# comprna/riser

Measured on NVIDIA B200. Metric: reads classified/sec (4 s chunks), higher is better.
Workload: dtype f16+e4m3

## Files before the change

### riser_b200/csrc/common.cuh

```cuda
#pragma once

#include <cuda_runtime.h>
#include <cuda_fp16.h>
#include <cuda_fp8.h>
#include <stdint.h>
#include <stdio.h>
#include <stdarg.h>

#include "../../include/riser_b200.h"

namespace riser {

inline char* err_buf() {
  static thread_local char buf[512] = {0};
  return buf;
}
inline int fail(int code, const char* fmt, ...) {
  va_list ap;
  va_start(ap, fmt);
  vsnprintf(err_buf(), 512, fmt, ap);
  va_end(ap);
  return code;
}
#define RISER_CUDA_TRY(expr)                                                              \
// ... 69 lines not shown
#define RISER_SPIN_NS 0
#endif
__device__ __forceinline__ void mbar_wait_relaxed(uint64_t* bar, uint32_t parity) {
  while (!mbar_try_wait(bar, parity)) {
    if (RISER_SPIN_NS > 0) __nanosleep(RISER_SPIN_NS);
  }
}

__device__ __forceinline__ void tma_prefetch_desc(const void* tmap) {
  asm volatile("prefetch.tensormap [%0];" ::"l"(reinterpret_cast<uint64_t>(tmap)) : "memory");
}
__device__ __forceinline__ void tma_load_2d(void* smem_dst, const void* tmap, uint64_t* bar,
                                            int32_t c0, int32_t c1) {
  asm volatile(
      "cp.async.bulk.tensor.2d.shared::cluster.global.mbarrier::complete_tx::bytes "
      "[%0], [%1, {%3, %4}], [%2];"
      ::"r"(smem_u32(smem_dst)), "l"(reinterpret_cast<uint64_t>(tmap)), "r"(smem_u32(bar)),
      "r"(c0), "r"(c1)
      : "memory");
}

__device__ __forceinline__ void bulk_prefetch_l2(const void* gsrc, uint32_t bytes) {
  asm volatile("cp.async.bulk.prefetch.L2.global [%0], %1;" ::"l"(reinterpret_cast<uint64_t>(gsrc)), "r"(bytes)
               : "memory");
}

__device__ __forceinline__ void bulk_load_1d(void* smem_dst, const void* gsrc, uint32_t bytes, uint64_t* bar) {
  asm volatile(
      "cp.async.bulk.shared::cluster.global.mbarrier::complete_tx::bytes [%0], [%1], %2, [%3];"
      ::"r"(smem_u32(smem_dst)), "l"(reinterpret_cast<uint64_t>(gsrc)), "r"(bytes), "r"(smem_u32(bar))
      : "memory");
}

__device__ __forceinline__ void tmem_alloc(uint32_t* smem_slot, uint32_t cols) {
  asm volatile("tcgen05.alloc.cta_group::1.sync.aligned.shared::cta.b32 [%0], %1;"
               ::"r"(smem_u32(smem_slot)), "r"(cols)
               : "memory");
}
__device__ __forceinline__ void tmem_relinquish() {
  asm volatile("tcgen05.relinquish_alloc_permit.cta_group::1.sync.aligned;" ::: "memory");
}
__device__ __forceinline__ void tmem_dealloc(uint32_t taddr, uint32_t cols) {
  asm volatile("tcgen05.dealloc.cta_group::1.sync.aligned.b32 %0, %1;" ::"r"(taddr), "r"(cols)
               : "memory");
}
__device__ __forceinline__ void tc_fence_before() {
  asm volatile("tcgen05.fence::before_thread_sync;" ::: "memory");
}
__device__ __forceinline__ void tc_fence_after() {
  asm volatile("tcgen05.fence::after_thread_sync;" ::: "memory");
}
__device__ __forceinline__ void umma_f16(uint32_t tmem_d, uint64_t desc_a, uint64_t desc_b,
                                         uint32_t idesc, uint32_t accumulate) {
  asm volatile(
      "{\n\t.reg .pred p;\n\t"
      "setp.ne.b32 p, %4, 0;\n\t"
      "tcgen05.mma.cta_group::1.kind::f16 [%0], %1, %2, %3, p;\n\t}\n"
      ::"r"(tmem_d), "l"(desc_a), "l"(desc_b), "r"(idesc), "r"(accumulate)
      : "memory");
}
__device__ __forceinline__ void umma_f8(uint32_t tmem_d, uint64_t desc_a, uint64_t desc_b,
                                        uint32_t idesc, uint32_t accumulate) {
  asm volatile(
      "{\n\t.reg .pred p;\n\t"
      "setp.ne.b32 p, %4, 0;\n\t"
      "tcgen05.mma.cta_group::1.kind::f8f6f4 [%0], %1, %2, %3, p;\n\t}\n"
// ... 202 lines not shown
```

### riser_b200/csrc/convnet.cu

```cuda
#include "common.cuh"

#include <cuda.h>

#include <algorithm>
#include <cmath>
#include <cstdio>
#include <cstdlib>
#include <cstring>
#include <memory>
#include <vector>

namespace riser {
namespace {

#ifndef RISER_DBG
#define RISER_DBG 0
#endif
#ifndef RISER_UNIFORM_ISSUE
#define RISER_UNIFORM_ISSUE 1
#endif
constexpr int kMaxLayers = 16;
constexpr int kBlockM = 128;
constexpr int kBlockK = 64;
constexpr int kMaxNTile = 256;
// ... 121 lines not shown
  int fused_prev = 0;
  Eo2Args eo2;
  size_t eo2_smem = 0;
  ConvArgs args;
  int n_supers_total = 0;
  int rows_per_super = 0;
  int flag_off = 0;
  size_t smem = 0;
};

}
}

struct riser_plan {
  const riser_model* model = nullptr;
  int B = 0, max_len = 0;
  int fuse_l0 = 0;
  uint8_t* flags = nullptr;
  riser::ActivityArgs activity;
  int chunk_reads = 0, n_chunked = 0;
  int Lmax[riser::kMaxLayers + 1];
  int Lp[riser::kMaxLayers + 1];
  size_t act_off[riser::kMaxLayers + 1];
  char* ws = nullptr;
  riser::LayerPlan layer[riser::kMaxLayers];
};

namespace riser {
namespace {

constexpr float kF8AScale = 1.f / 8.f;
constexpr float kF8LoScale = 512.f;
template <int N>
__device__ __forceinline__ void store_f8_planes(const float (&r)[N], const __half2 (&h)[N / 2], uint8_t* a8,
                                                int lo_stride) {
  uint32_t pa[N / 4], pl[N / 4];
#pragma unroll
  for (int j = 0; j < N / 4; ++j) {
    uint32_t wa[2], wl[2];
#pragma unroll
    for (int e = 0; e < 2; ++e) {
      const int c = 4 * j + 2 * e;
      const float2 back = __half22float2(h[c / 2]);
      wa[e] = __nv_cvt_float2_to_fp8x2(make_float2(r[c] * kF8AScale, r[c + 1] * kF8AScale), __NV_SATFINITE,
                                       __NV_E4M3);
      wl[e] = __nv_cvt_float2_to_fp8x2(make_float2((r[c] - back.x) * kF8LoScale, (r[c + 1] - back.y) * kF8LoScale),
                                       __NV_SATFINITE, __NV_E4M3);
    }
    pa[j] = wa[0] | (wa[1] << 16);
    pl[j] = wl[0] | (wl[1] << 16);
  }
  if (N == 8) {
    *reinterpret_cast<uint2*>(a8) = make_uint2(pa[0], pa[1]);
    *reinterpret_cast<uint2*>(a8 + lo_stride) = make_uint2(pl[0], pl[1]);
  } else {
#pragma unroll
    for (int j = 0; j < N / 16; ++j) {
      *reinterpret_cast<uint4*>(a8 + 16 * j) = make_uint4(pa[4 * j], pa[4 * j + 1], pa[4 * j + 2], pa[4 * j + 3]);
      *reinterpret_cast<uint4*>(a8 + lo_stride + 16 * j) =
          make_uint4(pl[4 * j], pl[4 * j + 1], pl[4 * j + 2], pl[4 * j + 3]);
    }
  }
}

__global__ void __launch_bounds__(256)
layer0_kernel(const float* __restrict__ x, int64_t ld_x, const int32_t* __restrict__ len0,
              const float* __restrict__ w, const float* __restrict__ bias, __half* __restrict__ out,
              int B, int Lp1, int cout, int cout_p, int planes, int f8) {
  __shared__ float sw[64 * 3];
  __shared__ float sb[64];
  for (int i = threadIdx.x; i < cout_p * 3; i += blockDim.x) sw[i] = (i < cout * 3) ? w[i] : 0.f;
  for (int i = threadIdx.x; i < cout_p; i += blockDim.x) sb[i] = (i < cout) ? bias[i] : 0.f;
  __syncthreads();
  const uint32_t groups = cout_p >> 3;
  const uint32_t total = static_cast<uint32_t>(B) * Lp1 * groups;
  for (uint32_t idx = blockIdx.x * blockDim.x + threadIdx.x; idx < total; idx += gridDim.x * blockDim.x) {
    const uint32_t r = idx / groups;
    const int c8 = static_cast<int>(idx - r * groups);
    const int b = static_cast<int>(r / static_cast<uint32_t>(Lp1));
    const int tp = static_cast<int>(r - static_cast<uint32_t>(b) * Lp1);
    const int L = len0[b];
    uint4* o = reinterpret_cast<uint4*>(out + static_cast<int64_t>(r) * cout_p * planes) + c8;
    uint8_t* o8 = reinterpret_cast<uint8_t*>(out) + static_cast<int64_t>(r) * cout_p * 4 + 2 * cout_p + c8 * 8;
    if (tp >= (L >> 1)) {
// ... 585 lines not shown
  }
  if (ms == 4) return pick_conv_planes<4, false, false, K32>(planes, wplanes);
  if (ms == 2) return pick_conv_planes<2, false, false, K32>(planes, wplanes);
  return pick_conv_planes<1, false, false, K32>(planes, wplanes);
}
template <bool K32>
ConvKernelFn pick_conv_f8(int ms, int resident) {
  if (resident) {
    if (ms == 4) return conv_tc_kernel<4, 1, 1, true, false, K32, true>;
    if (ms == 2) return conv_tc_kernel<2, 1, 1, true, false, K32, true>;
    return conv_tc_kernel<1, 1, 1, true, false, K32, true>;
  }
  if (ms == 4) return conv_tc_kernel<4, 1, 1, false, false, K32, true>;
  if (ms == 2) return conv_tc_kernel<2, 1, 1, false, false, K32, true>;
  return conv_tc_kernel<1, 1, 1, false, false, K32, true>;
}
ConvKernelFn pick_conv_kernel(int ms, int planes, int wplanes, int resident, int fused = 0, int k32 = 0,
                              int f8 = 0) {
  if (f8) return k32 ? pick_conv_f8<true>(ms, resident) : pick_conv_f8<false>(ms, resident);
  return k32 ? pick_conv_k<true>(ms, planes, wplanes, resident, fused)
             : pick_conv_k<false>(ms, planes, wplanes, resident, fused);
}

constexpr int kF2Pairs = 255;
#ifndef RISER_F2_CVT_WARPS
#define RISER_F2_CVT_WARPS 6
#endif
constexpr int kF2Threads = 576 + 32 * RISER_F2_CVT_WARPS;
constexpr uint32_t kF2A1Tile = 264 * 64;
constexpr uint32_t kF2A0Tile = 256 * 64;
constexpr int kF2N0 = 48;
constexpr int kF2D0Col = 256;
constexpr int kF2CvtThreads = 32 * RISER_F2_CVT_WARPS;
constexpr int kF2XStages = 4;
constexpr int kF2MaxLocalItems = 2048;
constexpr uint32_t kF2XStage = 260 * 16;

struct F2Smem {
  uint64_t w_full;
  uint64_t x_full[kF2XStages], x_empty[kF2XStages];
  uint64_t a0_full[2], a0_empty[2];
  uint64_t d0_full[2], d0_empty[2];
  uint64_t a1_full[2], a1_empty[2];
  uint64_t d1_full[2], d1_empty[2][2];
  uint32_t tmem_base;
  alignas(16) float bias[32];
  uint8_t my_flags[kF2MaxLocalItems];
};

struct F2Iter {
  const uint8_t* local;
  int i, item, n_items, step;
  __device__ __forceinline__ F2Iter(const uint8_t* l, int n) : local(l), i(0), item(blockIdx.x), n_items(n), step(gridDim.x) {}
  __device__ __forceinline__ int take() {
    while (item < n_items) {
      const int cur = item;
      const bool f = local ? (local[i] != 0) : true;
      item += step;
      ++i;
      if (f) return cur;
    }
    return -1;
  }
};

__device__ __forceinline__ uint32_t h2_bits(__half2 h) { return *reinterpret_cast<uint32_t*>(&h); }

template <int MODE>
__global__ void __launch_bounds__(kF2Threads, 1)
fused01_kernel(const __grid_constant__ CUtensorMap tm_b, const __grid_constant__ CUtensorMap tm_b8, const ConvArgs a) {
  extern __shared__ unsigned char smem_dyn[];
  unsigned char* base = smem_dyn + ((1024u - (smem_u32(smem_dyn) & 1023u)) & 1023u);
  constexpr bool F8 = (MODE == 3);
  constexpr bool KC = (MODE == 4);
  constexpr int PLANES = (MODE >= 2) ? 2 : 1;
  constexpr int WPLANES = (MODE == 1 || MODE == 2) ? 2 : 1;
  constexpr uint32_t kW1Bytes = KC ? 3 * 32 * 128 : (F8 ? 2 : WPLANES) * 3 * 32 * 64;
  constexpr uint32_t kB0Bytes = kF2N0 * 64;
  constexpr uint32_t kA1Stage = PLANES * 2 * kF2A1Tile;
  unsigned char* w1 = base;
  unsigned char* b0 = w1 + kW1Bytes;
  unsigned char* a0_ring = b0 + kB0Bytes;
  unsigned char* a1_ring = a0_ring + 2 * kF2A0Tile;
  unsigned char* x_ring = a1_ring + 2 * kA1Stage;
  F2Smem& s = *reinterpret_cast<F2Smem*>(x_ring + kF2XStages * kF2XStage);

  const int warp = uniform_warp_id();
  const int lane = threadIdx.x & 31;
  const int n_items = a.n_supers;
  const int n_pairs = a.rows_in >> 1;
  const uint8_t* flags0 = a.flags ? a.flags + a.super0 : nullptr;
  const uint8_t* flags_l = flags0 ? s.my_flags : nullptr;

  if (threadIdx.x == 0) {
    tma_prefetch_desc(&tm_b);
    mbar_init(&s.w_full, 1);
    for (int i = 0; i < kF2XStages; ++i) {
      mbar_init(&s.x_full[i], 1);
      mbar_init(&s.x_empty[i], kF2CvtThreads / 32);
    }
    for (int i = 0; i < 2; ++i) {
      mbar_init(&s.a0_full[i], kF2CvtThreads / 32);
      mbar_init(&s.a0_empty[i], 1);
      mbar_init(&s.d0_full[i], 1);
      mbar_init(&s.d0_empty[i], 4);
      mbar_init(&s.a1_full[i], 8);
      mbar_init(&s.a1_empty[i], 1);
      mbar_init(&s.d1_full[i], 1);
      mbar_init(&s.d1_empty[i][0], 4);
      mbar_init(&s.d1_empty[i][1], 4);
    }
    fence_mbar_init();
  }
  if (warp == 1) {
    tmem_alloc(&s.tmem_base, kTmemCols);
    tmem_relinquish();
  }
  for (uint32_t i = threadIdx.x; i < (2 * kF2A0Tile + 2 * kA1Stage + kF2XStages * kF2XStage) / 16; i += kF2Threads)
// ... 5 lines not shown
  if (threadIdx.x < kF2N0) {
    const int n = threadIdx.x, c = n % 24, odd = n / 24;
    float w[3] = {0.f, 0.f, 0.f}, bb = 0.f;
    if (c < a.cout0) {
      w[0] = a.w0[c * 3];
      w[1] = a.w0[c * 3 + 1];
      w[2] = a.w0[c * 3 + 2];
      bb = a.b0[c];
    }
    __half kh[4], kl[4];
#pragma unroll
    for (int k = 0; k < 4; ++k) kh[k] = kl[k] = __float2half_rn(0.f);
#pragma unroll
    for (int tap = 0; tap < 3; ++tap) {
      const __half h = __float2half_rn(w[tap]);
      kh[tap + odd] = h;
      kl[tap + odd] = __float2half_rn(w[tap] - __half2float(h));
    }
    const __half bh = __float2half_rn(bb), bl = __float2half_rn(bb - __half2float(bh));
    __half c0[8] = {kh[0], kh[1], kh[2], kh[3], kh[0], kh[1], kh[2], kh[3]};
    __half c1[8] = {kl[0], kl[1], kl[2], kl[3], bh, bl, __float2half_rn(0.f), __float2half_rn(0.f)};
    const int sw = (n >> 1) & 3;
    *reinterpret_cast<uint4*>(b0 + n * 64 + ((0 ^ sw) << 4)) = *reinterpret_cast<const uint4*>(c0);
    *reinterpret_cast<uint4*>(b0 + n * 64 + ((1 ^ sw) << 4)) = *reinterpret_cast<const uint4*>(c1);
  }
  asm volatile("fence.proxy.async.shared::cta;" ::: "memory");
  tc_fence_before();
  __syncthreads();
  tc_fence_after();
  const uint32_t tmem_base = s.tmem_base;

  if (warp == 0) {
    if (lane == 0) {
      mbar_arrive_expect_tx(&s.w_full, kW1Bytes);
      if (KC) {
        for (int tap = 0; tap < 3; ++tap) tma_load_2d(w1 + (2 - tap) * 4096, &tm_b, &s.w_full, 0, tap * a.cout_p);
      } else {
        for (int wp = 0; wp < WPLANES; ++wp)
          for (int tap = 0; tap < 3; ++tap)
            tma_load_2d(w1 + (wp * 3 + 2 - tap) * 2048, &tm_b, &s.w_full, 0, (wp * 3 + tap) * a.cout_p);
      }
      if (F8)
        for (int tap = 0; tap < 3; ++tap)
          tma_load_2d(w1 + (3 + 2 - tap) * 2048, &tm_b8, &s.w_full, 0, tap * a.cout_p);
      const int t_max = static_cast<int>(a.ld_x >> 2);
      F2Iter iter(flags_l, n_items);
      int k = 0;
      for (int item = iter.take(); item >= 0; item = iter.take(), ++k) {
        const int st = k % kF2XStages;
        mbar_wait(&s.x_empty[st], ((k / kF2XStages) & 1) ^ 1);
        unsigned char* dst = x_ring + st * kF2XStage;
        long long u_lo = static_cast<long long>(a.super0 + item) * kF2Pairs - 2;
        long long u_hi = u_lo + 258;
        const int i_lo = (u_lo < 0) ? static_cast<int>(-u_lo) - 2 : -2;
        if (u_lo < 0) u_lo = 0;
        if (u_hi > n_pairs - 1) u_hi = n_pairs - 1;
        uint32_t bytes[2] = {0, 0};
        const float* src[2] = {nullptr, nullptr};
        int slot[2] = {0, 0};
        if (u_hi >= u_lo) {
          const int b = static_cast<int>((static_cast<unsigned long long>(static_cast<uint32_t>(u_lo)) * a.pair_magic) >> 40);
          const int t0 = static_cast<int>(u_lo) - b * a.half_lp;
          const int n_total = static_cast<int>(u_hi - u_lo) + 1;
          const int n_first = min(n_total, a.half_lp - t0);
          const int n1 = max(0, min(n_first, t_max - t0));
          src[0] = a.x + static_cast<long long>(b) * a.ld_x + 4 * t0;
          slot[0] = i_lo + 2;
          bytes[0] = 16u * n1;
          const int n2 = max(0, min(n_total - n_first, t_max));
          src[1] = a.x + static_cast<long long>(b + 1) * a.ld_x;
          slot[1] = i_lo + 2 + n_first;
          bytes[1] = 16u * n2;
        }
        mbar_arrive_expect_tx(&s.x_full[st], bytes[0] + bytes[1]);
        if (bytes[0]) bulk_load_1d(dst + 16 * slot[0], src[0], bytes[0], &s.x_full[st]);
        if (bytes[1]) bulk_load_1d(dst + 16 * slot[1], src[1], bytes[1], &s.x_full[st]);
      }
    }
  } else if (warp == 1) {
    const bool leader = RISER_UNIFORM_ISSUE ? elect_one() : (lane == 0);
    if (RISER_UNIFORM_ISSUE || lane == 0) {
      mbar_wait(&s.w_full, 0);
      tc_fence_after();
      const uint32_t w1_addr = smem_u32(w1), b0_addr = smem_u32(b0);
      const uint32_t a0_addr = smem_u32(a0_ring), a1_addr = smem_u32(a1_ring);
      const uint32_t idesc0 = umma_idesc_f16(kBlockM, kF2N0);
      const uint32_t idesc64 = umma_idesc_f16(kBlockM, 64);
      const uint64_t db0 = sw_desc<true>(b0_addr);
      F2Iter iter(flags_l, n_items);
      int k0 = 0;
      auto issue_layer0 = [&]() {
        const int st = k0 & 1;
        mbar_wait(&s.a0_full[st], (k0 >> 1) & 1);
        tc_fence_after();
#pragma unroll
        for (int h = 0; h < 2; ++h) {
          mbar_wait(&s.d0_empty[h], (k0 & 1) ^ 1);
          tc_fence_after();
          if (leader) {
#pragma unroll
            for (int sub = 0; sub < 2; ++sub)
              umma_f16(tmem_base + kF2D0Col + (h * 2 + sub) * kF2N0,
                       sw_desc<true>(a0_addr + st * kF2A0Tile + sub * 128 * 64) + 2 * h, db0, idesc0, 0);
          }
          umma_commit_p(leader, &s.d0_full[h]);
        }
        umma_commit_p(leader, &s.a0_empty[st]);
        ++k0;
      };
      int cur = iter.take();
      if (cur >= 0) issue_layer0();
      int k1 = 0;
      while (cur >= 0) {
        const int nxt = iter.take();
        if (nxt >= 0) issue_layer0();
        const int st = k1 & 1;
        mbar_wait(&s.a1_full[st], (k1 >> 1) & 1);
        tc_fence_after();
        const uint32_t a1s = a1_addr + st * kA1Stage;
#pragma unroll
        for (int sub = 0; sub < 2; ++sub) {
          mbar_wait(&s.d1_empty[st][sub], ((k1 >> 1) & 1) ^ 1);
          tc_fence_after();
        }
        auto issue_group = [&](uint32_t a_tiles, uint32_t w_set, bool f8, bool first) {
          if (!leader) return;
#pragma unroll
          for (int tap = 0; tap < 3; ++tap) {
#pragma unroll
            for (int k = 0; k < 2; ++k) {
              const uint64_t db = sw_desc<true>(w_set + (2 - tap) * 2048) + 2 * k;
#pragma unroll
              for (int sub = 0; sub < 2; ++sub) {
#pragma unroll
                for (int pe = 0; pe < 2; ++pe) {
                  const int par = (pe == 0) ? ((tap == 1) ? 0 : 1) : ((tap == 1) ? 1 : 0);
                  const int shift = (pe == 0) ? ((tap == 2) ? 1 : 0) : ((tap == 0) ? 0 : 1);
                  const uint64_t da = sw_desc<true>(a_tiles + par * kF2A1Tile + (sub * 128 + shift) * 64) + 2 * k;
                  const uint32_t d = tmem_base + st * 128 + (2 * sub + pe) * 32;
                  if ((RISER_DBG & 1) && !(first && tap == 0 && k == 0)) continue;
                  if (f8) umma_f8(d, da, db, a.idesc, 1);
                  else umma_f16(d, da, db, a.idesc, !(first && tap == 0 && k == 0));
                }
              }
            }
          }
        };
        if (KC) {
          if (leader) {
#pragma unroll
            for (int k = 0; k < 4; ++k) {
              const uint64_t w21 = sw_desc<false>(w1_addr) + 2 * k;
              const uint64_t w10 = sw_desc<false>(w1_addr + 4096) + 2 * k;
              const uint64_t w0 = sw_desc<false>(w1_addr + 8192) + 2 * k;
#pragma unroll
              for (int sub = 0; sub < 2; ++sub) {
                const uint32_t e_rows = a1s + sub * 128 * 128, o_rows = e_rows + 2 * kF2A1Tile;
                const uint32_t d_even = tmem_base + st * 128 + 2 * sub * 32, d_odd = d_even + 32;
                umma_f16(d_even, sw_desc<false>(e_rows) + 2 * k, w10, idesc64, k != 0);
                umma_f16(d_even, sw_desc<false>(o_rows + 128) + 2 * k, w21, idesc64, 1);
                umma_f16(d_even, sw_desc<false>(o_rows) + 2 * k, w0, a.idesc, 1);
                umma_f16(d_odd, sw_desc<false>(e_rows + 128) + 2 * k, w21, a.idesc, 1);
              }
            }
          }
        } else {
#pragma unroll
        for (int wp = 0; wp < WPLANES; ++wp)
#pragma unroll
          for (int ap = 0; ap < ((wp == 0 && !F8) ? PLANES : 1); ++ap)
            issue_group(a1s + ap * 2 * kF2A1Tile, w1_addr + wp * 3 * 2048, false, wp == 0 && ap == 0);
        }
        if (F8)
          issue_group(a1s + 2 * kF2A1Tile, w1_addr + 3 * 2048, true, false);
        umma_commit_p(leader, &s.a1_empty[st]);
        umma_commit_p(leader, &s.d1_full[st]);
        ++k1;
        cur = nxt;
      }
    }
  } else if (warp < 2 + kF2CvtThreads / 32) {
    const int ct = (warp - 2) * 32 + lane;
    const __half2 one2 = __floats2half2_rn(1.f, 1.f);
    F2Iter iter(flags_l, n_items);
    int k = 0;
    for (int item = iter.take(); item >= 0; item = iter.take(), ++k) {
      const int st = k & 1;
      const int xst = k % kF2XStages;
      mbar_wait_relaxed(&s.x_full[xst], (k / kF2XStages) & 1);
      mbar_wait_relaxed(&s.a0_empty[st], ((k >> 1) & 1) ^ 1);
      unsigned char* tile = a0_ring + st * kF2A0Tile;
      const float* xs = reinterpret_cast<const float*>(x_ring + xst * kF2XStage) + 8;
      const long long u0 = static_cast<long long>(a.super0 + item) * kF2Pairs;
      for (int i = ct - 1; i <= 255 && !(RISER_DBG & 32); i += kF2CvtThreads) {
        const long long u = u0 + i;
        const bool inb = (u >= 0 && u < n_pairs);
        const uint32_t uu = inb ? static_cast<uint32_t>(u) : 0u;
        const int b = static_cast<int>((static_cast<unsigned long long>(uu) * a.pair_magic) >> 40);
        const int t4 = 4 * (static_cast<int>(uu) - b * a.half_lp);
        const int L = inb ? __ldg(a.len0 + b) : 0;
        const float4 x03 = *reinterpret_cast<const float4*>(xs + 4 * i);
        const float2 x01 = make_float2(x03.x, x03.y), x23 = make_float2(x03.z, x03.w);
        float xm1 = (t4 > 0) ? xs[4 * i - 1] : 0.f;
        float x4 = xs[4 * i + 4];
        const int half_len = L >> 1;
        const bool e_ok = (t4 >> 1) < half_len;
        const bool o_ok = (t4 >> 1) + 1 < half_len;
        float x2 = (t4 + 2 < L) ? x23.x : 0.f;
        if (t4 + 4 >= L) x4 = 0.f;
        auto clampf = [](float v) { return fminf(fmaxf(v, -65504.f), 65504.f); };
        const float v[6] = {clampf(xm1), clampf(x01.x), clampf(x01.y), clampf(x2), clampf(x23.y), clampf(x4)};
        __half2 hi[3], lo[3];
#pragma unroll
        for (int j = 0; j < 3; ++j) {
          hi[j] = __floats2half2_rn(v[2 * j], v[2 * j + 1]);
          const float2 back = __half22float2(hi[j]);
          lo[j] = __floats2half2_rn(v[2 * j] - back.x, v[2 * j + 1] - back.y);
        }
        if (i >= 0) {
          unsigned char* row = tile + i * 64;
          const int sw = (i >> 1) & 3;
          uint4 c0 = make_uint4(0, 0, 0, 0), c1 = make_uint4(0, 0, 0, 0);
          if (e_ok) {
            c0 = make_uint4(h2_bits(hi[0]), h2_bits(hi[1]), h2_bits(lo[0]), h2_bits(lo[1]));
            c1 = make_uint4(h2_bits(hi[0]), h2_bits(hi[1]), h2_bits(one2), 0u);
          }
          *reinterpret_cast<uint4*>(row + ((0 ^ sw) << 4)) = c0;
          *reinterpret_cast<uint4*>(row + ((1 ^ sw) << 4)) = c1;
        }
        if (i + 1 <= 255) {
          unsigned char* row = tile + (i + 1) * 64;
          const int sw = ((i + 1) >> 1) & 3;
          uint4 c2 = make_uint4(0, 0, 0, 0), c3 = make_uint4(0, 0, 0, 0);
          if (o_ok) {
            c2 = make_uint4(h2_bits(hi[1]), h2_bits(hi[2]), h2_bits(lo[1]), h2_bits(lo[2]));
            c3 = make_uint4(h2_bits(hi[1]), h2_bits(hi[2]), h2_bits(one2), 0u);
          }
          *reinterpret_cast<uint4*>(row + ((2 ^ sw) << 4)) = c2;
          *reinterpret_cast<uint4*>(row + ((3 ^ sw) << 4)) = c3;
        }
      }
      asm volatile("fence.proxy.async.shared::cta;" ::: "memory");
      __syncwarp();
      if (lane == 0) {
        mbar_arrive(&s.x_empty[xst]);
        mbar_arrive(&s.a0_full[st]);
      }
    }
  } else if (warp < 10 + kF2CvtThreads / 32) {
    const int q = warp & 3;
    const int h = (warp - 2 - kF2CvtThreads / 32) >> 2;
    F2Iter iter(flags_l, n_items);
    int k = 0;
    for (int item = iter.take(); item >= 0; item = iter.take(), ++k) {
      const int st = k & 1;
      mbar_wait_relaxed(&s.a1_empty[st], ((k >> 1) & 1) ^ 1);
      mbar_wait_relaxed(&s.d0_full[h], k & 1);
      tc_fence_after();
      unsigned char* tile_hi = a1_ring + st * kA1Stage + h * kF2A1Tile;
#pragma unroll
      for (int sub = 0; sub < 2; ++sub) {
        const uint32_t taddr = tmem_base + (static_cast<uint32_t>(32 * q) << 16) + kF2D0Col + (h * 2 + sub) * kF2N0;
        uint32_t e0[16], e1[8], o0[16], o1[8];
        if (RISER_DBG & 4) {
#pragma unroll
          for (int j = 0; j < 16; ++j) e0[j] = o0[j] = 0u;
#pragma unroll
          for (int j = 0; j < 8; ++j) e1[j] = o1[j] = 0u;
        } else {
        tmem_ld_32x16(taddr, e0);
        tmem_ld_32x16(taddr + 24, o0);
        }
        if (RISER_DBG & 4) {
        } else if (a.cout0 > 20) {
          tmem_ld_32x8(taddr + 16, e1);
          tmem_ld_32x8(taddr + 40, o1);
        } else {
#pragma unroll
          for (int j = 4; j < 8; ++j) e1[j] = o1[j] = 0u;
          tmem_ld_32x4(taddr + 16, e1);
          tmem_ld_32x4(taddr + 40, o1);
        }
        tmem_ld_wait();
        if (sub == 1) {
          tc_fence_before();
          __syncwarp();
          if (lane == 0) mbar_arrive(&s.d0_empty[h]);
        }
        if (RISER_DBG & 16) continue;
        const int row = sub * 128 + 32 * q + lane;
// ... 37 lines not shown
          }
#pragma unroll
          for (int c8 = 0; c8 < 3; ++c8)
            *reinterpret_cast<uint4*>(rp + 2 * kF2A1Tile + ((c8 ^ sw) << 4)) = *reinterpret_cast<const uint4*>(lv + 4 * c8);
        }
        if (F8) {
          uint32_t pa[6], pl[6];
#pragma unroll
          for (int j = 0; j < 6; ++j) {
            uint32_t wa[2], wl[2];
#pragma unroll
            for (int e = 0; e < 2; ++e) {
              const int c = 4 * j + 2 * e;
              const float2 back = __half22float2(hv[c / 2]);
              wa[e] = __nv_cvt_float2_to_fp8x2(make_float2(v[c] * kF8AScale, v[c + 1] * kF8AScale), __NV_SATFINITE,
                                               __NV_E4M3);
              wl[e] = __nv_cvt_float2_to_fp8x2(
                  make_float2((v[c] - back.x) * kF8LoScale, (v[c + 1] - back.y) * kF8LoScale), __NV_SATFINITE, __NV_E4M3);
            }
            pa[j] = wa[0] | (wa[1] << 16);
            pl[j] = wl[0] | (wl[1] << 16);
          }
          unsigned char* rp8 = rp + 2 * kF2A1Tile;
          *reinterpret_cast<uint4*>(rp8 + ((0 ^ sw) << 4)) = make_uint4(pa[0], pa[1], pa[2], pa[3]);
          *reinterpret_cast<uint4*>(rp8 + ((1 ^ sw) << 4)) = make_uint4(pa[4], pa[5], 0u, 0u);
          *reinterpret_cast<uint4*>(rp8 + ((2 ^ sw) << 4)) = make_uint4(pl[0], pl[1], pl[2], pl[3]);
          *reinterpret_cast<uint4*>(rp8 + ((3 ^ sw) << 4)) = make_uint4(pl[4], pl[5], 0u, 0u);
        }
      }
      asm volatile("fence.proxy.async.shared::cta;" ::: "memory");
      __syncwarp();
      if (lane == 0) mbar_arrive(&s.a1_full[st]);
    }
  } else {
    const int q = warp & 3;
    const int sub = (warp - 10 - kF2CvtThreads / 32) >> 2;
    const int row_elems = a.cout_p * a.out_planes;
    const int lo_off = (a.out_planes == 2 && !a.out_f8) ? a.cout_p : 0;
    const float inv_scale = a.w_inv_scale;
    F2Iter iter(flags_l, n_items);
    int k = 0;
    for (int item = iter.take(); item >= 0; item = iter.take(), ++k) {
      const int st = k & 1;
      const int j = sub * 128 + 32 * q + lane;
      const long long u = static_cast<long long>(a.super0 + item) * kF2Pairs + j;
      const bool ok = (j < kF2Pairs) && (u < n_pairs);
      const uint32_t uu = ok ? static_cast<uint32_t>(u) : 0u;
      const int b = static_cast<int>((static_cast<unsigned long long>(uu) * a.pair_magic) >> 40);
      const int tp = static_cast<int>(uu) - b * a.half_lp;
      const bool valid = ok && tp < (__ldg(a.len0 + b) >> a.shift);
      const bool writable = ok && tp < a.Lp_out;
      const int64_t out_row = a.out_eo ? static_cast<int64_t>(tp & 1) * a.n_pairs_out + static_cast<int64_t>(b) * a.half_lp_out + (tp >> 1)
                                       : static_cast<int64_t>(b) * a.Lp_out + tp;
      __half* orow = static_cast<__half*>(a.out) + out_row * row_elems;
      mbar_wait_relaxed(&s.d1_full[st], (k >> 1) & 1);
      tc_fence_after();
      const uint32_t taddr = tmem_base + (static_cast<uint32_t>(32 * q) << 16) + st * 128 + 2 * sub * 32;
      auto finish = [&](int c16, const float (&m)[16]) {
        if (!(writable && !((RISER_DBG & 2) && a.Lp_out > 0))) return;
        float r[16];
        if (valid) {
#pragma unroll
          for (int c4 = 0; c4 < 4; ++c4) {
            const float4 bb = *reinterpret_cast<const float4*>(&s.bias[c16 * 16 + c4 * 4]);
            const float bv[4] = {bb.x, bb.y, bb.z, bb.w};
#pragma unroll
            for (int e = 0; e < 4; ++e) {
              const int c = c4 * 4 + e;
              r[c] = fmaxf(fmaf(m[c], inv_scale, bv[e]), 0.f);
            }
          }
        } else {
#pragma unroll
          for (int c = 0; c < 16; ++c) r[c] = 0.f;
        }
        __half2 hv[8];
#pragma unroll
        for (int c = 0; c < 8; ++c) hv[c] = sat_half2(r[2 * c], r[2 * c + 1]);
        st_global_256(orow + c16 * 16, *reinterpret_cast<const uint4*>(hv), *reinterpret_cast<const uint4*>(hv + 4));
        if (lo_off) {
          __half2 lv[8];
#pragma unroll
          for (int c = 0; c < 8; ++c) {
            const float2 back = __half22float2(hv[c]);
            lv[c] = __floats2half2_rn(r[2 * c] - back.x, r[2 * c + 1] - back.y);
          }
          st_global_256(orow + lo_off + c16 * 16, *reinterpret_cast<const uint4*>(lv),
                        *reinterpret_cast<const uint4*>(lv + 4));
        }
        if (a.out_f8)
          store_f8_planes<16>(r, hv, reinterpret_cast<uint8_t*>(orow) + 2 * a.cout_p + c16 * 16, a.cout_p);
      };
      float m0[16];
      {
        uint32_t ve[16], vo[16];
        if (RISER_DBG & 8) {
#pragma unroll
          for (int j = 0; j < 16; ++j) ve[j] = vo[j] = 0u;
        } else {
          tmem_ld_32x16(taddr, ve);
          tmem_ld_32x16(taddr + 32, vo);
        }
        tmem_ld_wait();
#pragma unroll
        for (int j = 0; j < 16; ++j) m0[j] = fmaxf(__uint_as_float(ve[j]), __uint_as_float(vo[j]));
      }
      uint32_t ve1[16], vo1[16];
      if (RISER_DBG & 8) {
#pragma unroll
        for (int j = 0; j < 16; ++j) ve1[j] = vo1[j] = 0u;
      } else {
        tmem_ld_32x16(taddr + 16, ve1);
        tmem_ld_32x16(taddr + 32 + 16, vo1);
      }
      finish(0, m0);
      tmem_ld_wait();
      tc_fence_before();
      __syncwarp();
      if (lane == 0) mbar_arrive(&s.d1_empty[st][sub]);
#pragma unroll
      for (int j = 0; j < 16; ++j) m0[j] = fmaxf(__uint_as_float(ve1[j]), __uint_as_float(vo1[j]));
      finish(1, m0);
      __syncwarp();
    }
  }

  tc_fence_before();
  __syncthreads();
  if (warp == 1) {
    tc_fence_after();
    tmem_dealloc(tmem_base, kTmemCols);
  }
}

typedef void (*FusedKernelFn)(const CUtensorMap, const CUtensorMap, const ConvArgs);
FusedKernelFn pick_fused01(int mode) {
  if (mode == 0) return fused01_kernel<0>;
  if (mode == 1) return fused01_kernel<1>;
  if (mode == 2) return fused01_kernel<2>;
  if (mode == 4) return fused01_kernel<4>;
  return fused01_kernel<3>;
}
size_t fused01_smem(int planes, int wplanes) {
  return 1024 + static_cast<size_t>(wplanes) * 3 * 32 * 64 + kF2N0 * 64 + 2 * kF2A0Tile +
         2 * static_cast<size_t>(planes) * 2 * kF2A1Tile + kF2XStages * kF2XStage + sizeof(F2Smem) + 64;
}

constexpr uint32_t kEoTile = 136 * 64;

template <int MS, int PLANES, int WPLANES>
__global__ void __launch_bounds__(64 + 128 * kMaxEpiSets, 1)
conv_eo_kernel(const __grid_constant__ CUtensorMap tm_e, const __grid_constant__ CUtensorMap tm_o,
               const __grid_constant__ CUtensorMap tm_b, const ConvArgs a) {
  extern __shared__ unsigned char smem_dyn[];
  unsigned char* base = smem_dyn + ((1024u - (smem_u32(smem_dyn) & 1023u)) & 1023u);
  constexpr uint32_t kGroup = MS * PLANES * 2 * kEoTile;
  const uint32_t b_bytes = a.n_tile * 64;
  unsigned char* a_ring = base;
  unsigned char* b_region = base + static_cast<size_t>(a.a_stages) * kGroup;
  const size_t b_region_bytes = static_cast<size_t>(WPLANES) * a.k_blocks * 3 * b_bytes;
  ConvSmem& s = *reinterpret_cast<ConvSmem*>(b_region + b_region_bytes);

  const int warp = uniform_warp_id();
  const int lane = threadIdx.x & 31;
  const int n_items = a.n_supers;
  const int acc2 = a.acc_cols;

  if (warp == 0 && lane == 0) {
    tma_prefetch_desc(&tm_e);
    tma_prefetch_desc(&tm_o);
    tma_prefetch_desc(&tm_b);
    for (int i = 0; i < a.a_stages; ++i) {
      mbar_init(&s.a_full[i], 1);
      mbar_init(&s.a_empty[i], 1);
    }
    mbar_init(&s.w_full, 1);
    for (int i = 0; i < a.acc_stages; ++i) {
      mbar_init(&s.tmem_full[i], 1);
// ... 1276 lines not shown
            break;
          }
        }
      }
    } else {
      a.resident = 0;
      a.ms = (2 * a.acc_cols <= kTmemCols) ? max_ms : 1;
      if (max_ms == 2 && 4 * a.acc_cols <= kTmemCols && 2 * 4 * a_group1 + 3 * b_bytes <= avail &&
          env_int("RISER_CONV_MS4_STREAM", 1))
        a.ms = 4;
      while (a.ms > 1 && 2 * a.ms * a_group1 + 2 * b_bytes > avail) a.ms >>= 1;
      const size_t a_group = a.ms * a_group1;
      int a_st = 2;
      int b_st = static_cast<int>((avail - a_st * a_group) / b_bytes);
      if (b_st > 4 && (a_st + 1) * a_group + 4 * b_bytes <= avail) {
        a_st = 3;
        b_st = static_cast<int>((avail - a_st * a_group) / b_bytes);
      }
      a.a_stages = a_st;
      a.b_stages = std::max(2, std::min(kMaxBStages, b_st));
      lp.smem = fixed + static_cast<size_t>(a.a_stages) * a_group + static_cast<size_t>(a.b_stages) * b_bytes;
    }
    a.acc_stages = std::max(1, std::min(kMaxAccStages, kTmemCols / (a.ms * a.acc_cols)));
    a.dual = (a.ms == 2 && !a.resident && env_int("RISER_DUAL_ISSUE", 1)) ? 1 : 0;
    a.epi_sets = (i == 1 && p->fuse_l0) ? 2 : std::max(2, std::min(env_int("RISER_EPI_SETS", kMaxEpiSets), 4));
    lp.rows_per_super = a.ms * kBlockM;
    if (fuse2) {
      p->fuse_l0 = 2;
      a.w0 = m->layer[0].w0;
      a.b0 = m->layer[0].bias;
      a.cout0 = m->layer[0].cout;
      lp.rows_per_super = 2 * kF2Pairs;
      lp.smem = fused01_smem(m->act_planes, L.f8 ? 2 : L.passes);
      a.planes = m->act_planes;
      if (L.wkc && m->layer[0].cout <= 20 && env_int("RISER_KC", 1)) {
        lp.kc = 1;
        const int st3 = make_tmap(&lp.tm_b, L.wkc, 64, 3ull * L.cout_p, 32, false);
        if (st3) return st3;
      }
    }
    if (lp.eo) {
      const uint64_t n_pairs = static_cast<uint64_t>(rows_in) / 2;
      const uint64_t pitch = static_cast<uint64_t>(L.cin_p) * m->act_planes;
      int st2 = make_tmap(&lp.tm_a, p->ws + p->act_off[i], pitch, n_pairs, 136, true);
      if (!st2) st2 = make_tmap(&lp.tm_a8, p->ws + p->act_off[i] + n_pairs * pitch * 2, pitch, n_pairs, 136, true);
      if (st2) return st2;
      a.acc_cols = round_up(2 * L.n_tile, 32);
      const size_t w_eo = static_cast<size_t>(L.passes) * a.k_blocks * 3 * b_bytes;
      const size_t group1 = static_cast<size_t>(m->act_planes) * 2 * kEoTile;
      a.ms = (2 * 2 * a.acc_cols <= kTmemCols && w_eo + 2 * 2 * group1 <= avail && env_int("RISER_EO_MS", 2) >= 2) ? 2 : 1;
      a.resident = 1;
      a.a_stages = std::min<int>(kMaxAStages, static_cast<int>((avail - w_eo) / (a.ms * group1)));
      a.acc_stages = std::max(1, std::min(kMaxAccStages, kTmemCols / (a.ms * a.acc_cols)));
      a.epi_sets = 4;
      lp.smem = fixed + w_eo + static_cast<size_t>(a.a_stages) * a.ms * group1;
      lp.rows_per_super = a.ms * 2 * kBlockM;
    }
    if (L.f8 && !a.resident && !k32 && !lp.eo && (L.n_tile % 16) == 0 && env_int("RISER_PAIR", 1) &&
        (i >= env_int("RISER_PAIR_FROM", 6) ||
         (L.n_tiles == 1 && static_cast<size_t>(3) * a.k_blocks * (L.cout_p / 2) * 128 + 3 * 136 * 128 <= avail &&
          env_int("RISER_PAIR_RESIDENT", 1)))) {
      lp.pair = 1;
      char ntile_key[32];
      snprintf(ntile_key, sizeof ntile_key, "RISER_PAIR_NTILE_L%d", i);
      const int wide = std::max(64, std::min(kMaxNTile, env_int(ntile_key, env_int("RISER_PAIR_NTILE", kMaxNTile))) & ~15);
      a.n_tile = std::min(wide, L.cout_p);
// ... 129 lines not shown

extern "C" int riser_forward_launches(const riser_plan* p) {
  if (!p) return 0;
  const int n = p->model->n_layers;
  const int chunks = p->n_chunked > 0 ? (p->B + p->chunk_reads - 1) / p->chunk_reads : 0;
  const int l0 = p->fuse_l0 ? (p->n_chunked > 0 ? chunks : 1) : 0;
  int fused = 0;
  for (int i = 1; i < n; ++i) fused += p->layer[i].fused_prev;
  return chunks * p->n_chunked + (n - p->n_chunked) + 1 - l0 - fused + (p->flags ? 1 : 0);
}

extern "C" int riser_plan_fused_layer0(const riser_plan* p) { return p ? p->fuse_l0 : 0; }

extern "C" int riser_plan_layer_eo(const riser_plan* p, int i) {
  return (p && i >= 1 && i < p->model->n_layers) ? p->layer[i].eo : 0;
}

extern "C" int riser_plan_layer_format(const riser_plan* p, int i) {
  if (!p || i < 1 || i >= p->model->n_layers) return 0;
  if (p->layer[i].fused_prev) return -1;
  if (p->model->layer[i].f8) return 3;
  return p->model->act_planes == 2 ? 2 : 1;
}

extern "C" int riser_plan_layer_kernel(const riser_plan* p, int i) {
  if (!p || i < 1 || i >= p->model->n_layers) return -1;
  if (i == 1 && p->fuse_l0 == 2) return 3;
  if (i == 1 && p->fuse_l0 == 1) return 4;
  if (p->layer[i].pair) return 2;
  if (p->layer[i].fuse_next || p->layer[i].fused_prev) return 5;
  return p->layer[i].eo ? 1 : 0;
}

extern "C" int riser_plan_layer_info(const riser_plan* p, int i, int64_t* offset, int* rows_per_read,
                                     int* channels_padded, int* channels, int* n_tile) {
  RISER_REQUIRE(p && offset && rows_per_read && channels_padded && channels && n_tile,
                "riser_plan_layer_info: null pointer");
  RISER_REQUIRE(i >= 1 && i <= p->model->n_layers, "riser_plan_layer_info: layer %d out of range", i);
  *offset = static_cast<int64_t>(p->act_off[i]);
  *rows_per_read = p->Lp[i];
  *channels_padded = p->model->layer[i - 1].cout_p * (i == p->model->n_layers ? 1 : p->model->act_planes);
  *channels = p->model->layer[i - 1].cout;
  *n_tile = p->model->layer[i - 1].n_tile;
  return RISER_OK;
}

namespace riser {
namespace {

int launch_layer0(const riser_plan* p, const float* x, int64_t ld_x, const int32_t* len, int b0, int nb,
                  cudaStream_t st) {
  const riser_model* m = p->model;
  if (p->fuse_l0) return RISER_OK;
  const LayerPack& L = m->layer[0];
  const int64_t total = static_cast<int64_t>(nb) * p->Lp[1] * (L.cout_p / 8);
  const int grid = static_cast<int>(std::min<int64_t>((total + 255) / 256, static_cast<int64_t>(m->sm_count) * 32));
  __half* out = reinterpret_cast<__half*>(p->ws + p->act_off[1]) +
                static_cast<int64_t>(b0) * p->Lp[1] * L.cout_p * m->act_planes;
  layer0_kernel<<<grid, 256, 0, st>>>(x + static_cast<int64_t>(b0) * ld_x, ld_x, len + b0, L.w0, L.bias, out, nb,
                                      p->Lp[1], L.cout, L.cout_p, m->act_planes, m->layer[1].f8);
  RISER_CUDA_TRY(cudaGetLastError());
  return RISER_OK;
}

int launch_conv(const riser_plan* p, int i, const float* x, int64_t ld_x, const int32_t* len, int b0, int nb,
                cudaStream_t st) {
// ... 132 lines not shown
```

Measured before the change: 738,300.

## Stage fused01 epilogue rows in shared memory and write via bulk async stores

The fused layer0/1 epilogue warps now pack output rows (f16 hi/lo or fp8 planes) into a per-warp shared-memory staging buffer. Lane 0 then issues cp.async.bulk stores for each contiguous row group, replacing per-thread scattered 256-bit global stores. The goal is coalesced, asynchronous output writes that overlap with the next item. To free shared memory the x input ring drops from 4 to 3 stages, which may expose more producer latency. The change also adds compile-time-disabled wait-time instrumentation and smem/alignment checks.

```diff
diff --git a/riser_b200/csrc/common.cuh b/riser_b200/csrc/common.cuh
--- a/riser_b200/csrc/common.cuh
+++ b/riser_b200/csrc/common.cuh
@@ -125,6 +125,20 @@
       : "memory");
 }
 
+__device__ __forceinline__ void st_shared_128(uint32_t addr, const uint4& v) {
+  asm volatile("st.shared.v4.b32 [%0], {%1, %2, %3, %4};" ::"r"(addr), "r"(v.x), "r"(v.y), "r"(v.z), "r"(v.w)
+               : "memory");
+}
+
+__device__ __forceinline__ void bulk_store_1d(void* gdst, uint32_t smem_src, uint32_t bytes) {
+  asm volatile("cp.async.bulk.global.shared::cta.bulk_group [%0], [%1], %2;"
+               ::"l"(reinterpret_cast<uint64_t>(gdst)), "r"(smem_src), "r"(bytes)
+               : "memory");
+}
+__device__ __forceinline__ void bulk_commit() { asm volatile("cp.async.bulk.commit_group;" ::: "memory"); }
+__device__ __forceinline__ void bulk_wait_read_all() { asm volatile("cp.async.bulk.wait_group.read 0;" ::: "memory"); }
+__device__ __forceinline__ void bulk_wait_all() { asm volatile("cp.async.bulk.wait_group 0;" ::: "memory"); }
+
 __device__ __forceinline__ void tmem_alloc(uint32_t* smem_slot, uint32_t cols) {
   asm volatile("tcgen05.alloc.cta_group::1.sync.aligned.shared::cta.b32 [%0], %1;"
                ::"r"(smem_u32(smem_slot)), "r"(cols)
diff --git a/riser_b200/csrc/convnet.cu b/riser_b200/csrc/convnet.cu
--- a/riser_b200/csrc/convnet.cu
+++ b/riser_b200/csrc/convnet.cu
@@ -177,9 +177,8 @@
 constexpr float kF8AScale = 1.f / 8.f;
 constexpr float kF8LoScale = 512.f;
 template <int N>
-__device__ __forceinline__ void store_f8_planes(const float (&r)[N], const __half2 (&h)[N / 2], uint8_t* a8,
-                                                int lo_stride) {
-  uint32_t pa[N / 4], pl[N / 4];
+__device__ __forceinline__ void pack_f8(const float (&r)[N], const __half2 (&h)[N / 2], uint32_t (&pa)[N / 4],
+                                        uint32_t (&pl)[N / 4]) {
 #pragma unroll
   for (int j = 0; j < N / 4; ++j) {
     uint32_t wa[2], wl[2];
@@ -195,6 +194,12 @@
     pa[j] = wa[0] | (wa[1] << 16);
     pl[j] = wl[0] | (wl[1] << 16);
   }
+}
+template <int N>
+__device__ __forceinline__ void store_f8_planes(const float (&r)[N], const __half2 (&h)[N / 2], uint8_t* a8,
+                                                int lo_stride) {
+  uint32_t pa[N / 4], pl[N / 4];
+  pack_f8<N>(r, h, pa, pl);
   if (N == 8) {
     *reinterpret_cast<uint2*>(a8) = make_uint2(pa[0], pa[1]);
     *reinterpret_cast<uint2*>(a8 + lo_stride) = make_uint2(pl[0], pl[1]);
@@ -846,9 +851,39 @@
 constexpr int kF2N0 = 48;
 constexpr int kF2D0Col = 256;
 constexpr int kF2CvtThreads = 32 * RISER_F2_CVT_WARPS;
-constexpr int kF2XStages = 4;
+constexpr int kF2XStages = 3;
 constexpr int kF2MaxLocalItems = 2048;
 constexpr uint32_t kF2XStage = 260 * 16;
+constexpr uint32_t kF2OutRow = 128;
+constexpr uint32_t kF2OutStage = 8 * 32 * kF2OutRow;
+
+#ifndef RISER_F2_WAITS
+#define RISER_F2_WAITS 0
+#endif
+enum F2Wait {
+  kF2wProdX, kF2wProdAll,
+  kF2wCvtX, kF2wCvtA0, kF2wCvtAll,
+  kF2wMmaA0, kF2wMmaA1, kF2wMmaD1, kF2wMmaOther, kF2wMmaAll,
+  kF2wMidA1, kF2wMidD0, kF2wMidAll,
+  kF2wEpiD1, kF2wEpiLd, kF2wEpiMath, kF2wEpiSt, kF2wEpiAll,
+  kF2wSlots
+};
+#if RISER_F2_WAITS
+__device__ unsigned long long g_f2_waits[kF2wSlots];
+#define F2W_DECL long long f2w[kF2wSlots] = {}; const long long f2w_t0 = clock64()
+#define F2W_TIME(slot, ...) do { const long long f2w_s = clock64(); __VA_ARGS__; f2w[slot] += clock64() - f2w_s; } while (0)
+#define F2W_MARK(var) const long long var = clock64()
+#define F2W_SPAN(slot, from) (f2w[slot] += clock64() - (from))
+#define F2W_FLUSH(all) do { f2w[all] = clock64() - f2w_t0;                                              \
+    if ((threadIdx.x & 31) == 0) for (int f2w_i = 0; f2w_i < kF2wSlots; ++f2w_i)                          \
+      if (f2w[f2w_i]) atomicAdd(&g_f2_waits[f2w_i], static_cast<unsigned long long>(f2w[f2w_i])); } while (0)
+#else
+#define F2W_DECL
+#define F2W_TIME(slot, ...) do { __VA_ARGS__; } while (0)
+#define F2W_MARK(var)
+#define F2W_SPAN(slot, from)
+#define F2W_FLUSH(all)
+#endif
 
 struct F2Smem {
   uint64_t w_full;
@@ -897,7 +932,8 @@
   unsigned char* a0_ring = b0 + kB0Bytes;
   unsigned char* a1_ring = a0_ring + 2 * kF2A0Tile;
   unsigned char* x_ring = a1_ring + 2 * kA1Stage;
-  F2Smem& s = *reinterpret_cast<F2Smem*>(x_ring + kF2XStages * kF2XStage);
+  unsigned char* out_stage = x_ring + kF2XStages * kF2XStage;
+  F2Smem& s = *reinterpret_cast<F2Smem*>(out_stage + kF2OutStage);
 
   const int warp = uniform_warp_id();
   const int lane = threadIdx.x & 31;
@@ -969,6 +1005,7 @@
 
   if (warp == 0) {
     if (lane == 0) {
+      F2W_DECL;
       mbar_arrive_expect_tx(&s.w_full, kW1Bytes);
       if (KC) {
         for (int tap = 0; tap < 3; ++tap) tma_load_2d(w1 + (2 - tap) * 4096, &tm_b, &s.w_full, 0, tap * a.cout_p);
@@ -985,7 +1022,7 @@
       int k = 0;
       for (int item = iter.take(); item >= 0; item = iter.take(), ++k) {
         const int st = k % kF2XStages;
-        mbar_wait(&s.x_empty[st], ((k / kF2XStages) & 1) ^ 1);
+        F2W_TIME(kF2wProdX, mbar_wait(&s.x_empty[st], ((k / kF2XStages) & 1) ^ 1));
         unsigned char* dst = x_ring + st * kF2XStage;
         long long u_lo = static_cast<long long>(a.super0 + item) * kF2Pairs - 2;
         long long u_hi = u_lo + 258;
@@ -1013,11 +1050,13 @@
         if (bytes[0]) bulk_load_1d(dst + 16 * slot[0], src[0], bytes[0], &s.x_full[st]);
         if (bytes[1]) bulk_load_1d(dst + 16 * slot[1], src[1], bytes[1], &s.x_full[st]);
       }
+      F2W_FLUSH(kF2wProdAll);
     }
   } else if (warp == 1) {
     const bool leader = RISER_UNIFORM_ISSUE ? elect_one() : (lane == 0);
     if (RISER_UNIFORM_ISSUE || lane == 0) {
-      mbar_wait(&s.w_full, 0);
+      F2W_DECL;
+      F2W_TIME(kF2wMmaOther, mbar_wait(&s.w_full, 0));
       tc_fence_after();
       const uint32_t w1_addr = smem_u32(w1), b0_addr = smem_u32(b0);
       const uint32_t a0_addr = smem_u32(a0_ring), a1_addr = smem_u32(a1_ring);
@@ -1028,11 +1067,11 @@
       int k0 = 0;
       auto issue_layer0 = [&]() {
         const int st = k0 & 1;
-        mbar_wait(&s.a0_full[st], (k0 >> 1) & 1);
+        F2W_TIME(kF2wMmaA0, mbar_wait(&s.a0_full[st], (k0 >> 1) & 1));
         tc_fence_after();
 #pragma unroll
         for (int h = 0; h < 2; ++h) {
-          mbar_wait(&s.d0_empty[h], (k0 & 1) ^ 1);
+          F2W_TIME(kF2wMmaOther, mbar_wait(&s.d0_empty[h], (k0 & 1) ^ 1));
           tc_fence_after();
           if (leader) {
 #pragma unroll
@@ -1052,12 +1091,12 @@
         const int nxt = iter.take();
         if (nxt >= 0) issue_layer0();
         const int st = k1 & 1;
-        mbar_wait(&s.a1_full[st], (k1 >> 1) & 1);
+        F2W_TIME(kF2wMmaA1, mbar_wait(&s.a1_full[st], (k1 >> 1) & 1));
         tc_fence_after();
         const uint32_t a1s = a1_addr + st * kA1Stage;
 #pragma unroll
         for (int sub = 0; sub < 2; ++sub) {
-          mbar_wait(&s.d1_empty[st][sub], ((k1 >> 1) & 1) ^ 1);
+          F2W_TIME(kF2wMmaD1, mbar_wait(&s.d1_empty[st][sub], ((k1 >> 1) & 1) ^ 1));
           tc_fence_after();
         }
         auto issue_group = [&](uint32_t a_tiles, uint32_t w_set, bool f8, bool first) {
@@ -1115,17 +1154,19 @@
         ++k1;
         cur = nxt;
       }
+      F2W_FLUSH(kF2wMmaAll);
     }
   } else if (warp < 2 + kF2CvtThreads / 32) {
     const int ct = (warp - 2) * 32 + lane;
     const __half2 one2 = __floats2half2_rn(1.f, 1.f);
+    F2W_DECL;
     F2Iter iter(flags_l, n_items);
     int k = 0;
     for (int item = iter.take(); item >= 0; item = iter.take(), ++k) {
       const int st = k & 1;
       const int xst = k % kF2XStages;
-      mbar_wait_relaxed(&s.x_full[xst], (k / kF2XStages) & 1);
-      mbar_wait_relaxed(&s.a0_empty[st], ((k >> 1) & 1) ^ 1);
+      F2W_TIME(kF2wCvtX, mbar_wait_relaxed(&s.x_full[xst], (k / kF2XStages) & 1));
+      F2W_TIME(kF2wCvtA0, mbar_wait_relaxed(&s.a0_empty[st], ((k >> 1) & 1) ^ 1));
       unsigned char* tile = a0_ring + st * kF2A0Tile;
       const float* xs = reinterpret_cast<const float*>(x_ring + xst * kF2XStage) + 8;
       const long long u0 = static_cast<long long>(a.super0 + item) * kF2Pairs;
@@ -1184,15 +1225,17 @@
         mbar_arrive(&s.a0_full[st]);
       }
     }
+    F2W_FLUSH(kF2wCvtAll);
   } else if (warp < 10 + kF2CvtThreads / 32) {
     const int q = warp & 3;
     const int h = (warp - 2 - kF2CvtThreads / 32) >> 2;
+    F2W_DECL;
     F2Iter iter(flags_l, n_items);
     int k = 0;
     for (int item = iter.take(); item >= 0; item = iter.take(), ++k) {
       const int st = k & 1;
-      mbar_wait_relaxed(&s.a1_empty[st], ((k >> 1) & 1) ^ 1);
-      mbar_wait_relaxed(&s.d0_full[h], k & 1);
+      F2W_TIME(kF2wMidA1, mbar_wait_relaxed(&s.a1_empty[st], ((k >> 1) & 1) ^ 1));
+      F2W_TIME(kF2wMidD0, mbar_wait_relaxed(&s.d0_full[h], k & 1));
       tc_fence_after();
       unsigned char* tile_hi = a1_ring + st * kA1Stage + h * kF2A1Tile;
 #pragma unroll
@@ -1296,12 +1339,16 @@
       __syncwarp();
       if (lane == 0) mbar_arrive(&s.a1_full[st]);
     }
+    F2W_FLUSH(kF2wMidAll);
   } else {
     const int q = warp & 3;
     const int sub = (warp - 10 - kF2CvtThreads / 32) >> 2;
-    const int row_elems = a.cout_p * a.out_planes;
-    const int lo_off = (a.out_planes == 2 && !a.out_f8) ? a.cout_p : 0;
+    const int row_bytes = 2 * a.cout_p * a.out_planes;
+    const bool wide = a.out_planes == 2;
     const float inv_scale = a.w_inv_scale;
+    unsigned char* stage = out_stage + (warp - 10 - kF2CvtThreads / 32) * 32 * kF2OutRow;
+    const uint32_t stage_addr = smem_u32(stage);
+    F2W_DECL;
     F2Iter iter(flags_l, n_items);
     int k = 0;
     for (int item = iter.take(); item >= 0; item = iter.take(), ++k) {
@@ -1316,8 +1363,18 @@
       const bool writable = ok && tp < a.Lp_out;
       const int64_t out_row = a.out_eo ? static_cast<int64_t>(tp & 1) * a.n_pairs_out + static_cast<int64_t>(b) * a.half_lp_out + (tp >> 1)
                                        : static_cast<int64_t>(b) * a.Lp_out + tp;
-      __half* orow = static_cast<__half*>(a.out) + out_row * row_elems;
-      mbar_wait_relaxed(&s.d1_full[st], (k >> 1) & 1);
+      const bool put = writable && !((RISER_DBG & 2) && a.Lp_out > 0);
+      const int grp = 2 * (b != __shfl_sync(0xffffffffu, b, 0)) + (a.out_eo ? (tp & 1) : 0);
+      uint32_t gmask[4];
+#pragma unroll
+      for (int g = 0; g < 4; ++g) gmask[g] = __ballot_sync(0xffffffffu, put && grp == g);
+      int slot = __popc(gmask[grp] & ((1u << lane) - 1u));
+#pragma unroll
+      for (int g = 0; g < 3; ++g) slot += (g < grp) ? __popc(gmask[g]) : 0;
+      const uint32_t srow = stage_addr + slot * row_bytes;
+      if (lane == 0) bulk_wait_read_all();
+      __syncwarp();
+      F2W_TIME(kF2wEpiD1, mbar_wait_relaxed(&s.d1_full[st], (k >> 1) & 1));
       tc_fence_after();
       const uint32_t taddr = tmem_base + (static_cast<uint32_t>(32 * q) << 16) + st * 128 + 2 * sub * 32;
       auto finish = [&](int c16, const float (&m)[16]) {
@@ -1341,22 +1398,48 @@
         __half2 hv[8];
 #pragma unroll
         for (int c = 0; c < 8; ++c) hv[c] = sat_half2(r[2 * c], r[2 * c + 1]);
-        st_global_256(orow + c16 * 16, *reinterpret_cast<const uint4*>(hv), *reinterpret_cast<const uint4*>(hv + 4));
-        if (lo_off) {
+        uint4 v[4];
+        uint32_t off[4];
+        v[0] = *reinterpret_cast<const uint4*>(hv);
+        v[1] = *reinterpret_cast<const uint4*>(hv + 4);
+        off[0] = 32 * c16;
+        off[1] = 32 * c16 + 16;
+        v[2] = v[3] = make_uint4(0, 0, 0, 0);
+        off[2] = off[3] = 0;
+        if (!wide) {
+        } else if (a.out_f8) {
+          uint32_t pa[4], pl[4];
+          pack_f8<16>(r, hv, pa, pl);
+          v[2] = make_uint4(pa[0], pa[1], pa[2], pa[3]);
+          v[3] = make_uint4(pl[0], pl[1], pl[2], pl[3]);
+          off[2] = 64 + 16 * c16;
+          off[3] = 96 + 16 * c16;
+        } else {
           __half2 lv[8];
 #pragma unroll
           for (int c = 0; c < 8; ++c) {
             const float2 back = __half22float2(hv[c]);
             lv[c] = __floats2half2_rn(r[2 * c] - back.x, r[2 * c + 1] - back.y);
           }
-          st_global_256(orow + lo_off + c16 * 16, *reinterpret_cast<const uint4*>(lv),
-                        *reinterpret_cast<const uint4*>(lv + 4));
-        }
-        if (a.out_f8)
-          store_f8_planes<16>(r, hv, reinterpret_cast<uint8_t*>(orow) + 2 * a.cout_p + c16 * 16, a.cout_p);
+          v[2] = *reinterpret_cast<const uint4*>(lv);
+          v[3] = *reinterpret_cast<const uint4*>(lv + 4);
+          off[2] = 64 + 32 * c16;
+          off[3] = 64 + 32 * c16 + 16;
+        }
+        F2W_MARK(f2w_st);
+        const int n = wide ? 4 : 2;
+#pragma unroll
+        for (int i = 0; i < 4; ++i) {
+          if (i >= n) break;
+          const int c = (i + lane) & (n - 1);
+          st_shared_128(srow + (c == 0 ? off[0] : c == 1 ? off[1] : c == 2 ? off[2] : off[3]),
+                        c == 0 ? v[0] : c == 1 ? v[1] : c == 2 ? v[2] : v[3]);
+        }
+        F2W_SPAN(kF2wEpiSt, f2w_st);
       };
       float m0[16];
       {
+        F2W_MARK(f2w_ld);
         uint32_t ve[16], vo[16];
         if (RISER_DBG & 8) {
 #pragma unroll
@@ -1366,6 +1449,7 @@
           tmem_ld_32x16(taddr + 32, vo);
         }
         tmem_ld_wait();
+        F2W_SPAN(kF2wEpiLd, f2w_ld);
 #pragma unroll
         for (int j = 0; j < 16; ++j) m0[j] = fmaxf(__uint_as_float(ve[j]), __uint_as_float(vo[j]));
       }
@@ -1377,16 +1461,34 @@
         tmem_ld_32x16(taddr + 16, ve1);
         tmem_ld_32x16(taddr + 32 + 16, vo1);
       }
-      finish(0, m0);
-      tmem_ld_wait();
+      F2W_TIME(kF2wEpiMath, finish(0, m0));
+      F2W_TIME(kF2wEpiLd, tmem_ld_wait());
       tc_fence_before();
       __syncwarp();
       if (lane == 0) mbar_arrive(&s.d1_empty[st][sub]);
 #pragma unroll
       for (int j = 0; j < 16; ++j) m0[j] = fmaxf(__uint_as_float(ve1[j]), __uint_as_float(vo1[j]));
-      finish(1, m0);
+      F2W_TIME(kF2wEpiMath, finish(1, m0));
+      F2W_MARK(f2w_cp);
+      asm volatile("fence.proxy.async.shared::cta;" ::: "memory");
       __syncwarp();
-    }
+      int64_t g_first[4];
+#pragma unroll
+      for (int g = 0; g < 4; ++g) g_first[g] = __shfl_sync(0xffffffffu, out_row, __ffs(gmask[g] | (1u << 31)) - 1);
+      if (lane == 0) {
+        uint32_t src = stage_addr;
+#pragma unroll
+        for (int g = 0; g < 4; ++g) {
+          const uint32_t bytes = __popc(gmask[g]) * row_bytes;
+          if (bytes) bulk_store_1d(static_cast<unsigned char*>(a.out) + g_first[g] * row_bytes, src, bytes);
+          src += bytes;
+        }
+        bulk_commit();
+      }
+      F2W_SPAN(kF2wEpiSt, f2w_cp);
+    }
+    if (lane == 0) bulk_wait_all();
+    F2W_FLUSH(kF2wEpiAll);
   }
 
   tc_fence_before();
@@ -1407,7 +1509,7 @@
 }
 size_t fused01_smem(int planes, int wplanes) {
   return 1024 + static_cast<size_t>(wplanes) * 3 * 32 * 64 + kF2N0 * 64 + 2 * kF2A0Tile +
-         2 * static_cast<size_t>(planes) * 2 * kF2A1Tile + kF2XStages * kF2XStage + sizeof(F2Smem) + 64;
+         2 * static_cast<size_t>(planes) * 2 * kF2A1Tile + kF2XStages * kF2XStage + kF2OutStage + sizeof(F2Smem) + 64;
 }
 
 constexpr uint32_t kEoTile = 136 * 64;
@@ -2750,6 +2852,12 @@
       a.cout0 = m->layer[0].cout;
       lp.rows_per_super = 2 * kF2Pairs;
       lp.smem = fused01_smem(m->act_planes, L.f8 ? 2 : L.passes);
+      RISER_REQUIRE(lp.smem <= static_cast<size_t>(max_smem), "fused01_kernel needs %zu bytes of shared memory, the device has %d",
+                    lp.smem, max_smem);
+      const size_t out_row_bytes = 2ull * a.cout_p * a.out_planes;
+      RISER_REQUIRE(out_row_bytes <= kF2OutRow && out_row_bytes % 16 == 0 &&
+                    (static_cast<size_t>(a.n_pairs_out) * out_row_bytes) % 16 == 0 &&
+                    (reinterpret_cast<uintptr_t>(a.out) & 15) == 0, "fused01_kernel: act_2 rows not 16-byte aligned");
       a.planes = m->act_planes;
       if (L.wkc && m->layer[0].cout <= 20 && env_int("RISER_KC", 1)) {
         lp.kc = 1;
@@ -2945,6 +3053,17 @@
   return p->layer[i].eo ? 1 : 0;
 }
 
+#if RISER_F2_WAITS
+extern "C" int riser_f2_waits(unsigned long long* out, int n) {
+  RISER_REQUIRE(out && n == riser::kF2wSlots, "riser_f2_waits: out[kF2wSlots]");
+  RISER_CUDA_TRY(cudaDeviceSynchronize());
+  RISER_CUDA_TRY(cudaMemcpyFromSymbol(out, riser::g_f2_waits, sizeof(unsigned long long) * n));
+  const unsigned long long zero[riser::kF2wSlots] = {};
+  RISER_CUDA_TRY(cudaMemcpyToSymbol(riser::g_f2_waits, zero, sizeof zero));
+  return RISER_OK;
+}
+#endif
+
 extern "C" int riser_plan_layer_info(const riser_plan* p, int i, int64_t* offset, int* rows_per_read,
                                      int* channels_padded, int* channels, int* n_tile) {
   RISER_REQUIRE(p && offset && rows_per_read && channels_padded && channels && n_tile,
```

Result: slower. 705,700 (median of 6 runs) (-4.4%).
